# openxrlab/xrsfm

Hardware: AMD Instinct MI355X
Metric: BA iterations/sec x (cams+points) (higher is better)
Workload: dtype f64; 1 GPU; synthetic BAL-style L: 1000 cams / 500000 points / 2000000 obs, GBA accurate (ba_solver.cc:626-629), seed 4; parallelism=single GPU, linear_solver=cholesky (explicit reduced camera matrix, exact)

## Files before the change

### include/xrsfm_ba.h

```cpp
#ifndef XRSFM_BA_H
#define XRSFM_BA_H

#include <stddef.h>
#include <stdint.h>

#ifdef __cplusplus
extern "C" {
#endif

#define XRSFM_BA_VERSION 1

#define XRSFM_BA_OK 0
#define XRSFM_BA_EINVAL (-1)
#define XRSFM_BA_ENODEV (-2)
#define XRSFM_BA_ENOMEM (-3)
#define XRSFM_BA_ECOMM (-4)
#define XRSFM_BA_ESTATE (-5)
#define XRSFM_BA_ETOOBIG (-6)
#define XRSFM_BA_EINTERNAL (-7)
#define XRSFM_BA_ESINGULAR (-8)

#define XRSFM_BA_SIMPLE_PINHOLE 0
#define XRSFM_BA_PINHOLE 1
#define XRSFM_BA_SIMPLE_RADIAL 2
// ... 201 lines not shown
int xrsfm_ba_profile_entry(xrsfm_ba_context *ctx, int index, const char **name, double *total_ms, int *launches);


int xrsfm_ba_debug_linearize(xrsfm_ba_context *ctx, double huber_a, int use_scaling, double *r, double *Jc,
                             double *Jp, double *Hpp, double *gp, double *Hcc_diag, double *gc, double *cost);

int xrsfm_ba_debug_schur_product(xrsfm_ba_context *ctx, double radius, const double *x, double *y, double *b);

int xrsfm_ba_debug_pack(const xrsfm_ba_problem *problem, int32_t stats[8], int32_t *slot_obs);

int xrsfm_ba_debug_sgroup(const xrsfm_ba_problem *problem, int G, int32_t stats[3], int32_t *pos_tile, int32_t *pos_code,
                          int32_t *tile_stride, int32_t *tile_cams, int32_t *tile_cidx, int32_t *cam_ptr_s);
int xrsfm_ba_debug_pack_gram(const xrsfm_ba_problem *problem, int32_t stats[8], int32_t *tile_ncam, uint8_t *slot_cidx,
                             int32_t *slot_campos_g);

int xrsfm_ba_debug_gram_schedule(int n_cams, int32_t *n_inst, int32_t *n_inst_all, uint16_t *entries);

int xrsfm_ba_debug_chol_plan(const xrsfm_ba_problem *problem, int32_t stats[8], int32_t *cam_offset, int32_t *facts);

int xrsfm_ba_debug_device_pack_check(const xrsfm_ba_problem *problem, int32_t *field, int32_t *index);

int xrsfm_ba_debug_set_block_pattern(xrsfm_ba_context *ctx, int n_pairs, const int32_t *row_col);

int xrsfm_ba_debug_cholesky_solve(xrsfm_ba_context *ctx, double radius, double *y, double *S_dense);

int xrsfm_ba_debug_reduced_system(xrsfm_ba_context *ctx, double radius, int32_t facts[16], int32_t *n_blocks, int32_t *blk_rc,
                                  double *blk, double *diag, double *b, double *y);

int xrsfm_ba_debug_wide(xrsfm_ba_context *ctx, double huber_a, double radius, double *cost, double *r, double *Jc, double *Jp,
                        double *Hcc_diag, double *gc, double *y);
// ... 14 lines not shown
```

### xrsfm_amd/capi.py

```python
from __future__ import annotations

import ctypes as C
import os

import numpy as np

from . import _build

_c_double_p = C.POINTER(C.c_double)
_c_int32_p = C.POINTER(C.c_int32)
_c_uint8_p = C.POINTER(C.c_uint8)


class CProblem(C.Structure):
    _fields_ = [
        ("n_cams", C.c_int32), ("n_points", C.c_int32), ("n_obs", C.c_int32), ("n_intr", C.c_int32),
        ("cam_q", _c_double_p), ("cam_t", _c_double_p), ("cam_const", _c_uint8_p), ("cam_intr", _c_int32_p),
        ("intr_model", _c_int32_p), ("intr_params", _c_double_p),
        ("points", _c_double_p), ("point_const", _c_uint8_p),
        ("obs_cam", _c_int32_p), ("obs_pt", _c_int32_p), ("obs_uv", _c_double_p),
    ]


class CPgProblem(C.Structure):
# ... 53 lines not shown
    ]

    def as_dict(self):
        return {f: getattr(self, f) for f, _ in self._fields_}


EXPORTS = [
    "xrsfm_ba_default_options", "xrsfm_ba_version", "xrsfm_ba_create", "xrsfm_ba_comm_unique_id",
    "xrsfm_ba_comm_init", "xrsfm_ba_run", "xrsfm_ba_reset", "xrsfm_ba_download", "xrsfm_ba_destroy",
    "xrsfm_ba_solve", "xrsfm_ba_filter_tracks", "xrsfm_ba_profile_entry", "xrsfm_ba_debug_linearize", "xrsfm_ba_debug_schur_product",
    "xrsfm_ba_debug_cholesky_solve", "xrsfm_ba_debug_set_block_pattern", "xrsfm_ba_debug_pack", "xrsfm_ba_debug_chol_plan", "xrsfm_ba_refine_pose", "xrsfm_ba_refine_pose_options", "xrsfm_ba_debug_comm_hook", "xrsfm_pg_default_options", "xrsfm_pg_solve", "xrsfm_ba_debug_pack_gram", "xrsfm_ba_debug_gram_schedule",
    "xrsfm_tag_default_options", "xrsfm_tag_refine", "xrsfm_ba_refine_poses", "xrsfm_ba_quiesce", "xrsfm_ba_debug_backsub", "xrsfm_ba_device_memory", "xrsfm_ba_download_intrinsics", "xrsfm_ba_debug_wide",
    "xrsfm_ba_debug_device_pack_check", "xrsfm_ba_warmup", "xrsfm_ba_debug_stored_j", "xrsfm_ba_debug_sgroup",
    "xrsfm_ba_debug_reduced_system", "xrsfm_ba_covariance", "xrsfm_ba_point_covariance", "xrsfm_ba_joint_covariance",
    "xrsfm_ba_map_covariance", "xrsfm_ba_debug_backsub_layout", "xrsfm_ba_run_batch", "xrsfm_ba_solve_batch",
    "xrsfm_ba_triangulate_options", "xrsfm_ba_triangulate_tracks",
]

CHOL_FACTS = ("T", "levels", "ordering", "schedule", "macro_levels", "split_levels", "la_depth", "fill_rest", "rest_apart", "packed",
              "bwd", "height_mask", "cw", "blocks", "n", "tiles_nz")
SCHEDULES = ("level", "panel", "lookahead")
BWD_FORMS = ("fused", "per_level", "all", "chunk", "push")


def _facts(v) -> dict:
    f = dict(zip(CHOL_FACTS, (int(x) for x in v)))
    f["schedule"] = SCHEDULES[f["schedule"]]
    f["bwd"] = BWD_FORMS[f["bwd"]]
    f["rest_apart"] = bool(f["rest_apart"]); f["packed"] = bool(f["packed"])
    f["heights"] = sorted(m * f["cw"] for m in range(1, 31) if (f["height_mask"] >> m) & 1)
    return f
# ... 490 lines not shown
          "xrsfm_ba_triangulate_tracks")
    return dict(points=points, status=status, inlier_mask=mask, num_inliers=ninl, num_trials=ntr, best_trial=best)


def debug_pack(problem: ProblemArrays) -> dict:
    stats = np.zeros(8, np.int32)
    slot_obs = np.full(problem.n_obs + 64 * (problem.n_points + 1), -2, np.int32)
    cs = problem.c_struct()
    check(load().xrsfm_ba_debug_pack(C.byref(cs), stats.ctypes.data_as(_c_int32_p), slot_obs.ctypes.data_as(_c_int32_p)), "xrsfm_ba_debug_pack")
    keys = ("tiles", "slots", "items", "regular_tiles", "long_items", "cam_entries", "longest_track", "active_points")
    out = dict(zip(keys, (int(v) for v in stats)))
    out["slot_obs"] = slot_obs[:out["slots"]].copy()
    return out


def debug_device_pack_check(problem: ProblemArrays) -> tuple:
    lib = load()
    lib.xrsfm_ba_debug_device_pack_check.argtypes = [C.POINTER(CProblem), _c_int32_p, _c_int32_p]
    lib.xrsfm_ba_debug_device_pack_check.restype = C.c_int
    f = np.zeros(1, np.int32); i = np.zeros(1, np.int32)
    cs = problem.c_struct()
    check(lib.xrsfm_ba_debug_device_pack_check(C.byref(cs), f.ctypes.data_as(_c_int32_p), i.ctypes.data_as(_c_int32_p)), "xrsfm_ba_debug_device_pack_check")
    return int(f[0]), int(i[0])


def debug_chol_plan(problem: ProblemArrays) -> dict:
    stats = np.zeros(8, np.int32)
    off = np.zeros(max(problem.n_cams, 1), np.int32)
    facts = np.zeros(16, np.int32)
    cs = problem.c_struct()
# ... 171 lines not shown
```

### xrsfm_amd/csrc/ba_chol.h

```cpp
#pragma once
#include "ba_kernels.h"
#include "ba_pack.h"

namespace xba {

constexpr int kNB = 64;
constexpr int kLdT = 66;
constexpr int kCamsPerTileDev = 10;

struct CholDev {
    int n, n_pad, T;
    double* S;
    const int* tmap; size_t ld; size_t tstride;
    double* Linv;
    double* y;
    double* rhs;
    double* x;
    const int* cam_off;
    const int* tile_rows;
    int cw, cpt;
};

__device__ __forceinline__ double* tile_ptr(const CholDev& c, int i, int k) {
    return c.tmap ? c.S + (size_t)c.tmap[i * c.T + k] * c.tstride : c.S + (size_t)(i * kNB) * c.ld + k * kNB;
// ... 286 lines not shown
                   int n_obs_pairs, double* __restrict__ scat2, double radius, double* __restrict__ pair_v = nullptr, int gram4 = 1,
                   const int* __restrict__ sgrp = nullptr, int n_list = 0, int wld = 0) {
    extern __shared__ __attribute__((aligned(16))) double smem_all[];
    constexpr bool MERGED = GRAM && NIK == 0;
    const int lane = MERGED ? (int)__builtin_amdgcn_mbcnt_hi(~0u, __builtin_amdgcn_mbcnt_lo(~0u, 0u)) : (int)threadIdx.x;
    const int wave = MERGED ? __builtin_amdgcn_readfirstlane((int)(threadIdx.x >> 6)) : 0;
    const int pos = MERGED ? (int)blockIdx.x * (int)(blockDim.x >> 6) + wave : (int)blockIdx.x;
    if (MERGED && pos >= n_list) return;
    double* const smem = smem_all + (size_t)wave * wld;
    XBA_STAMP(0, 0);
    SGroup sg{0, 1, smem, wld, 0.0, 0.0, -1};
    if (MERGED && sgrp) {
        const int code = __builtin_amdgcn_readfirstlane(sgrp[pos]);
        sg.idx = code & 15; sg.len = code >> 4;
    }
    const int entry = item_list[MERGED ? n_list - 1 - pos : pos];
    Item it;
    if (GRAM) { it.first_tile = entry; it.n_tiles = 1; }
    else it = d.items[entry];
    if (GRAM || it.n_tiles == 1) {
        int dt0 = -1, dt1 = -1;
        int g4_se = 0, g4_n = 0;
        if (GRAM) {
            const int C0 = d.tile_ncam[it.first_tile];
            const int* src = pair_dst + n_obs_pairs + d.tile_gt_off[it.first_tile];
            const int a0 = lane / kGramTabLd, b0 = lane - kGramTabLd * a0;
            const int a1 = (lane + kWave) / kGramTabLd, b1 = lane + kWave - kGramTabLd * a1;
            if (b0 > a0 && b0 < C0) dt0 = src[a0 * C0 + b0];
            if (b1 > a1 && b1 < C0 && a1 < kGramTabLd) dt1 = src[a1 * C0 + b1];
            if (NIK <= 2 && gram4) g4_se = gram4_sched_load<6>(C0, lane, g4_n);
        }
        const SlotCtx s = load_slot(d, it.first_tile, lane);
        const int cp = d.slot_campos_s[s.slot];
        const int cidx_raw = GRAM ? (int)d.slot_cidx[s.slot] : 0;
        const int L = d.tile_stride[it.first_tile];
        int g_pos = kWave - 1, g_pk0 = 0, g_pk1 = 0, g_pk2 = 0;
        if (GRAM && L == 0) {
            const int C0 = d.tile_ncam[it.first_tile];
            const int* trun = d.tile_run + (size_t)it.first_tile * kTileRunLd;
            const int c0 = lane / 14, c1 = (lane + 64) / 14, c2 = (lane + 128) / 14;
            g_pos = (int)d.slot_gpos[s.slot];
            if (c0 < C0) g_pk0 = trun[c0];
            if (c1 < C0) g_pk1 = trun[c1];
            if (c2 < C0) g_pk2 = trun[c2];
        }
        double V[18];
        int npair = 0, pbase = 0;
        {
            double o28[28];
            XBA_STAMP(0, 1);
            if (s.valid) {
                double hcv[6], gv[3];
                {
// ... 8 lines not shown
                if (PREP) { double hf[6]; point_factor(hcv, radius, hf);
#pragma unroll
                    for (int k = 0; k < 6; ++k) hcv[k] = hf[k]; }
                XBA_STAMP(0, 2);
                pairs_V<PREP>(F, E, hcv, V);
                XBA_STAMP(0, 3);
                pairs_diag<PREP>(F, V, hcv, gv, o28);
            } else if (PREP) { dead_values(V); dead_values(o28); }
            else {
#pragma unroll
                for (int k = 0; k < 18; ++k) V[k] = XBA_DEAD;
#pragma unroll
                for (int k = 0; k < 28; ++k) o28[k] = XBA_DEAD;
            }
            XBA_STAMP(0, 4);
            const int Cg = GRAM ? d.tile_ncam[it.first_tile] : 0;
            if (L > 0) {
                const int T = __popcll(__ballot(s.valid)) / L;
                double* red = smem;
#pragma unroll
                for (int h = 0; h < 2; ++h) {
#pragma unroll
                    for (int k = 0; k < 14; ++k) red[lane * kRedLd + k] = o28[14 * h + k];
                    __builtin_amdgcn_s_waitcnt(0xc07f);
                    __builtin_amdgcn_wave_barrier();
                    if ((L == 4 && T == 16) || (L == 2 && T == 32) || (L == 3 && T == 21)) {
                        const bool on = lane < 14 * L;
                        const int r = on ? lane / 14 : 0, k = lane - 14 * r;
                        const int cpr = __shfl(cp, r, kWave);
                        if (on) {
                            const double* src = red + r * kRedLd + k;
// ... 59 lines not shown
                            }
                            for (; j < n; ++j) sum += src[j * kRedLd];
                            d.scat[28 * (size_t)cpr + 14 * h + k] = sum;
                        }
                    }
                    __builtin_amdgcn_s_waitcnt(0xc07f);
                    __builtin_amdgcn_wave_barrier();
                }
            } else if (cp >= 0) {
                double2* out = reinterpret_cast<double2*>(d.scat + 28 * (size_t)cp);
#pragma unroll
                for (int k = 0; k < 14; ++k) out[k] = make_double2(o28[2 * k], o28[2 * k + 1]);
            }
        }
        XBA_STAMP(0, 5);
        const int C = d.tile_ncam[it.first_tile];
        if (GRAM) {
            const unsigned long long headmask = __ballot(s.head);
            const int T = __popcll(headmask);
            const int nvalid = __popcll(__ballot(s.valid));
            const int t = __popcll(headmask & ((2ull << lane) - 1ull)) - 1;
            const int cidx = s.valid ? cidx_raw : 0;
            int passes = 1;
            (void)gram_lds_need(C, T, &passes);
            const int Th = (T + passes - 1) / passes;
            const int R = 6 * C, Rp = (R + 15) & ~15, Cp = ((3 * Th + 3) & ~3) + kGramPad;
            double* Vst = smem;
            int* dtab = reinterpret_cast<int*>(smem + R * Cp);
            dtab[lane] = dt0;
            if (lane + kWave < kGramTabLd * kGramTabLd) dtab[lane + kWave] = dt1;
            const bool dense = nvalid == T * C;
            (void)Rp;
            unsigned short* sched = reinterpret_cast<unsigned short*>(dtab + kGramTabLd * kGramTabLd);
            if (NIK <= 2 && g4_n > 0 && passes == 1) {
                gram4_sched_store(sched, g4_se, lane, g4_n);
                gram_tile4<6>(Vst, R, Cp, C, dtab, scat2, lane, V, s.valid, t, cidx, T, dense, sched, g4_n, sg, d.scat);
// ... 1294 lines not shown
```

### xrsfm_amd/csrc/ba_kernels.h

```cpp
#pragma once
#include "ba_math.h"

namespace xba {

constexpr int kWave = 64;
constexpr int kBlock = 256;
constexpr int kWavesPerBlock = kBlock / kWave;

struct Item { int first_tile; int n_tiles; };

struct PcgStatus {
    double rz;
    double rr;
    double bb;
    double pq;
    int it;
    int done;
    unsigned arrived;
};

enum Scal {
    S_COST = 0, S_XNORM2_PTS, S_MODEL, S_STEP2_PTS, S_COST_CAND, S_STEP2_CAMS, S_XNORM2_CAMS,
    S_GRADMAX_PTS, S_GRADMAX_CAMS,
    S_BWD_ERR,
// ... 11 lines not shown
struct Dev {
    int n_cams, n_pts, n_tiles, n_slots, n_items;
    const int* slot_cam; const int* slot_pt; const int* slot_campos;
    const double* slot_u; const double* slot_v;
    const Item* items;
    const int* tile_stride;
    const int* tile_maxlen;
    const int* tile_ncam;
    const int* tile_gt_off;
    const unsigned char* slot_cidx;
    const int* slot_campos_g;
    const unsigned char* slot_gpos;
    const int* tile_run;
    const int* cam_ptr_g;
    const int* slot_campos_s; const int* cam_ptr_s;
    CamRec* cam; CamRec* cam_cand; const int* cam_model; const unsigned char* cam_const; const int* cam_ptr;
    double* cam_act;
    double* P; double* P_cand; const unsigned char* pt_const;
    double* scale_c; double* scale_p;
    double* rt; double* Jp;
    double huber_a;
    CamLin* camrec;
    double* Hpp; double* gp; double* Hinv;
    double* Hc;
    double* camlin;
    double* Dc2;
    double* camS;
    double* Minv;
    double* b;
    double* px; double* pr; double* pz; double* pp; double* pq;
    double* yp;
    double* scat;
    double* part;
    double* campart;
    double* ptpart;
    double* pcgpart;
    double* pcgW;
    double* pcgSW;
    double* pcgE;
    double* scal;
    PcgStatus* st;
};

#ifdef XBA_TIMELINE
__device__ unsigned long long g_stamps[3][64][16];
#define XBA_STAMP(kern, i) do { if ((threadIdx.x & 63) == 0 && (blockIdx.x % 97) == 0 && blockIdx.x / 97 < 64 && (threadIdx.x >> 6) == 0) g_stamps[kern][blockIdx.x / 97][i] = __builtin_readcyclecounter(); } while (0)
#define XBA_STAMP_W1(kern, i) do { if ((threadIdx.x & 63) == 0 && (blockIdx.x % 97) == 0 && blockIdx.x / 97 < 64 && (threadIdx.x >> 6) == 1) g_stamps[kern][blockIdx.x / 97][i] = __builtin_readcyclecounter(); } while (0)
#else
#define XBA_STAMP(kern, i) do {} while (0)
#define XBA_STAMP_W1(kern, i) do {} while (0)
#endif

#ifdef XBA_POISON
#define XBA_DEAD (__builtin_nan(""))
#define XBA_DEAD1 (__builtin_nan(""))
#define XBA_DEAD_VALUE(x) ((x) = __builtin_nan(""))
#else
#define XBA_DEAD 0.0
#define XBA_DEAD1 1.0
#define XBA_DEAD_VALUE(x) asm volatile("" : "=v"(x))
// ... 150 lines not shown
    bool valid, head;
};

__device__ __forceinline__ SlotCtx load_slot(const Dev& d, int tile, int lane) {
    SlotCtx s;
    s.lane = lane;
    s.slot = tile * kWave + lane;
    s.cam = d.slot_cam[s.slot];
    s.pt = d.slot_pt[s.slot];
    s.valid = s.cam >= 0;
    const int prev = __shfl_up(s.pt, 1, kWave);
    s.head = s.valid && (lane == 0 || prev != s.pt);
    return s;
}


__device__ __forceinline__ void robust_obs(const double (&M)[9], const double t[3], const double* intr, int model, const double Pw[3],
                                           double u, double v, double huber_a, Proj& pr, double& rho, double& sw) {
    project<true>(M, t, intr, model, Pw, u, v, pr);
    double rho1;
    rho = huber(pr.r0 * pr.r0 + pr.r1 * pr.r1, huber_a, rho1);
    sw = sqrt(rho1);
}

__device__ __forceinline__ void obs_rj(const Dev& d, int slot, int cam, const double (&M)[9], const double Pw[3],
                                       double& r0, double& r1, double (&j)[6]) {
    const CamRec& c = d.cam[cam];
    const double t[3] = {c.t[0], c.t[1], c.t[2]};
    Proj pr;
    double rho, sw;
// ... 83 lines not shown
    extern __shared__ __attribute__((aligned(16))) double lin_smem_acc[];
    double* acc = lin_smem_acc + (threadIdx.x >> 6) * (kWave * 13);
    if (is_long && lane == 0) {
#pragma unroll
        for (int k = 0; k < 9; ++k) acc[k] = 0.0;
    }
    double cost = 0.0, xn2 = 0.0, gm = 0.0;
    int long_pt = -1;
    for (int tl = 0; tl < (LONG ? it.n_tiles : 1); ++tl) {
        const SlotCtx s = load_slot(d, it.first_tile + tl, lane);
        const int cp = d.slot_campos_g[s.slot];
        const int tile = it.first_tile + tl;
        const int stride = d.tile_stride[tile];
        const int Cg = LONG ? 0 : d.tile_ncam[tile];
        const int maxlen = d.tile_maxlen[tile];
        double v[9] = {0, 0, 0, 0, 0, 0, 0, 0, 0};
        double cs[12] = {0, 0, 0, 0, 0, 0, 0, 0, 0, 0, 0, 0};
        double spk[3] = {XBA_DEAD1, XBA_DEAD1, XBA_DEAD1};
        if (s.valid) {
            const CamRec& c = d.cam[s.cam];
            double q[4] = {c.q[0], c.q[1], c.q[2], c.q[3]};
            double t[3] = {c.t[0], c.t[1], c.t[2]};
            const double* P = d.P + 3 * (size_t)s.pt;
            const double Pw[3] = {P[0], P[1], P[2]};
            double M[9];
            quat_to_mat(q, M);
            Proj pr;
            double rho, sw;
            robust_obs(M, t, c.intr, d.cam_model[s.cam], Pw, d.slot_u[s.slot], d.slot_v[s.slot], huber_a, pr, rho, sw);
            cost = cost + rho;
// ... 97 lines not shown
#pragma unroll
            for (int k = 0; k < 9; ++k) acc[k] += v[k];
        }
    }
    if (is_long && lane == 0 && long_pt >= 0) {
        double* H = d.Hpp + 6 * (size_t)long_pt;
#pragma unroll
        for (int k = 0; k < 6; ++k) H[k] = acc[k];
        double* g = d.gp + 3 * (size_t)long_pt;
        g[0] = acc[6]; g[1] = acc[7]; g[2] = acc[8];
        const double* sp = d.scale_p + 3 * (size_t)long_pt;
        gm = fmax(fabs(acc[6] / sp[0]), fmax(fabs(acc[7] / sp[1]), fabs(acc[8] / sp[2])));
    }
    cost = wave_sum(cost);
    xn2 = wave_sum(xn2);
#pragma unroll
    for (int off = 32; off > 0; off >>= 1) gm = fmax(gm, __shfl_xor(gm, off, kWave));
    if (lane == 0) { d.part[item] = cost; d.part[d.n_items + item] = xn2; d.part[2 * (size_t)d.n_items + item] = gm; }
}

__global__ __launch_bounds__(kBlock) __attribute__((amdgpu_waves_per_eu(4, 4))) void k_linearize(Dev d, double huber_a) {
    const int lane = threadIdx.x & (kWave - 1);
    const int item = __builtin_amdgcn_readfirstlane(blockIdx.x * kWavesPerBlock + (threadIdx.x >> 6));
    if (item >= d.n_items) return;
    const Item it = d.items[item];
    if (it.n_tiles > 1) linearize_item<true>(d, it, item, lane, huber_a);
    else linearize_item<false>(d, it, item, lane, huber_a);
}

__global__ __launch_bounds__(kBlock) void k_cost(Dev d, double huber_a) {
    const int lane = threadIdx.x & (kWave - 1);
    const int item = __builtin_amdgcn_readfirstlane(blockIdx.x * kWavesPerBlock + (threadIdx.x >> 6));
    if (item >= d.n_items) return;
    const Item it = d.items[item];
    double cost = 0.0;
    for (int tl = 0; tl < it.n_tiles; ++tl) {
        const int slot = (it.first_tile + tl) * kWave + lane;
        const int cam = d.slot_cam[slot];
        if (cam >= 0) {
            const CamRec& c = d.cam_cand[cam];
            double q[4] = {c.q[0], c.q[1], c.q[2], c.q[3]};
            double t[3] = {c.t[0], c.t[1], c.t[2]};
            const double* P = d.P_cand + 3 * (size_t)d.slot_pt[slot];
            const double Pw[3] = {P[0], P[1], P[2]};
            double M[9];
            quat_to_mat(q, M);
            Proj pr;
            project<false>(M, t, c.intr, d.cam_model[cam], Pw, d.slot_u[slot], d.slot_v[slot], pr);
            double rho1;
            cost += huber(pr.r0 * pr.r0 + pr.r1 * pr.r1, huber_a, rho1);
        }
    }
    cost = wave_sum(cost);
    if (lane == 0) d.part[item] = cost;
}

template <int K, bool WT = false>
__device__ __forceinline__ void segsum_body(const double* __restrict__ scat, const int* __restrict__ ptr, double* __restrict__ out, int c,
// ... 728 lines not shown
template <bool PREP>
#if XBA_BACKSUB_WAVES > 0
__global__ __launch_bounds__(kBlock) __attribute__((amdgpu_waves_per_eu(XBA_BACKSUB_WAVES, XBA_BACKSUB_WAVES)))
#else
__global__ __launch_bounds__(kBlock)
#endif
void k_backsub(Dev d, int n_item_blocks, CamLin* __restrict__ camrec_cand, double radius) {
    if ((int)blockIdx.x >= n_item_blocks) {
        const int c = (blockIdx.x - n_item_blocks) * kBlock + threadIdx.x;
        if (c < d.n_cams) cam_update_one(d, c, d.px + 6 * (size_t)c, camrec_cand);
        return;
    }
    const int lane = threadIdx.x & (kWave - 1);
    const int item = __builtin_amdgcn_readfirstlane(blockIdx.x * kWavesPerBlock + (threadIdx.x >> 6));
    if (item >= d.n_items) return;
    const Item it = d.items[item];
    double model = 0.0, step2 = 0.0;
    if (it.n_tiles == 1) {
        const SlotCtx s = load_slot(d, it.first_tile, lane);
        const int maxlen = d.tile_maxlen[it.first_tile];
        double E[6], v0, v1, r0, r1;
        double w[3] = {0, 0, 0};
        double hh[6], gg[3], spv[3], Pv[3];
        bool var = false;
        if (s.valid) {
            const double* h = (PREP ? d.Hpp : d.Hinv) + 6 * (size_t)s.pt;
            const double* g = d.gp + 3 * (size_t)s.pt;
            const double* sp = d.scale_p + 3 * (size_t)s.pt;
            const double* P = d.P + 3 * (size_t)s.pt;
#pragma unroll
            for (int k = 0; k < 6; ++k) hh[k] = h[k];
            gg[0] = g[0]; gg[1] = g[1]; gg[2] = g[2];
#pragma unroll
            for (int k = 0; k < 3; ++k) { spv[k] = sp[k]; Pv[k] = P[k]; }
            var = !d.pt_const[s.pt];
// ... 100 lines not shown
            if (cam >= 0) {
                const double* y = d.px + 6 * (size_t)cam;
                double F[12], E[6], r0, r1;
                load_FE_rc(d, slot, cam, pt0, F, E, r0, r1);
                double v0 = 0.0, v1 = 0.0;
#pragma unroll
                for (int k = 0; k < 6; ++k) { v0 += F[k] * y[k]; v1 += F[6 + k] * y[k]; }
                const double m0 = v0 + E[0] * u[0] + E[1] * u[1] + E[2] * u[2];
                const double m1 = v1 + E[3] * u[0] + E[4] * u[1] + E[5] * u[2];
                model += m0 * (r0 - 0.5 * m0) + m1 * (r1 - 0.5 * m1);
            }
        }
    }
    model = wave_sum(model);
    step2 = wave_sum(step2);
    if (lane == 0) { d.part[2 * d.n_items + item] = model; d.part[3 * d.n_items + item] = step2; }
}

__global__ void k_cam_update(Dev d) {
    const int c = blockIdx.x * blockDim.x + threadIdx.x;
    if (c >= d.n_cams) return;
    cam_update_one(d, c, d.px + 6 * (size_t)c, nullptr);
}

__device__ __forceinline__ double cam_gradmax_one(const Dev& d, int c, const double* g) {
    double m = 0.0;
    const unsigned cc = d.cam_const[c];
    const bool active = d.cam_act[c] > 0.0;
    const double* sc = d.scale_c + 6 * (size_t)c;
    if (active && !(cc & 1u)) {
// ... 188 lines not shown
```

### xrsfm_amd/csrc/xrsfm_ba.hip

```cpp
#include <dlfcn.h>
#include <hip/hip_runtime.h>

#include <algorithm>
#include <chrono>
#include <condition_variable>
#include <deque>
#include <cmath>
#include <cstdio>
#include <cstdlib>
#include <cstring>
#include <map>
#include <mutex>
#include <thread>
#include <type_traits>
#include <vector>

#include "../../include/xrsfm_ba.h"
#include "ba_chol.h"
#include "ba_cov.h"
#include "ba_filter.h"
#include "ba_kernels.h"
#include "ba_lba.h"
#include "ba_pack.h"
#include "ba_plan.h"
// ... 122 lines not shown
    int n_points_caller = 0;
    double* h_scal = nullptr;
    double* h_scal_dev = nullptr;
    unsigned long long seq = 0;
    PcgStatus* h_st = nullptr;
    void* comm = nullptr; int n_ranks = 1, rank = 0;
    xrsfm_ba_allreduce_fn hook = nullptr; void* hook_user = nullptr; std::vector<double> hook_buf;
    bool multi() const { return comm != nullptr || hook != nullptr; }
    bool profiling = false;
    std::vector<hipEvent_t> ev_pool; size_t ev_used = 0;
    struct Rec { int kid; size_t e0; int tag; };
    std::vector<Rec> recs;
    double prof_ms[K_COUNT] = {0}; int prof_n[K_COUNT] = {0};
    bool dev_packed = false; int host_pack_level = 2;
    int* dpk_slot_obs = nullptr; unsigned char* dpk_gt_cell = nullptr;
    bool linearized = false;
    unsigned long long debug_stall_ticks = 0;
    bool poisoned = false;
    bool fused = true;
    bool wide = false;
    DevW w{};
    std::vector<int> cam_intr_host;
    bool pcg_coarse = true; double* pcg_w = nullptr;
    bool prep_fused = true;
    double step_radius = 0.0;
    bool step_prep = false;
    bool step_valid = false;
    bool backsub_done = false;
    bool gradmax_done = false, published = false;
    double* part2 = nullptr; unsigned* ticket = nullptr;
// ... 515 lines not shown
    (void)hipFuncSetAttribute((const void*)k_schur_pairs<true, false, NI>, hipFuncAttributeMaxDynamicSharedMemorySize, pairs_max);
    XBA_PAIRS_ATTR(1) XBA_PAIRS_ATTR(2) XBA_PAIRS_ATTR(3) XBA_PAIRS_ATTR(4)
#undef XBA_PAIRS_ATTR
    {
        const int merged_max = std::max(pairs_max, kSGroupMax * (kGramSmallLds + 16));
        (void)hipFuncSetAttribute((const void*)k_schur_pairs<true, true, 0>, hipFuncAttributeMaxDynamicSharedMemorySize, merged_max);
        (void)hipFuncSetAttribute((const void*)k_schur_pairs<true, false, 0>, hipFuncAttributeMaxDynamicSharedMemorySize, merged_max);
    }
    (void)hipFuncSetAttribute((const void*)k_schur_pairs<false, true, 0>, hipFuncAttributeMaxDynamicSharedMemorySize, pairs_max);
    (void)hipFuncSetAttribute((const void*)k_schur_pairs<false, false, 0>, hipFuncAttributeMaxDynamicSharedMemorySize, pairs_max);
    (void)hipFuncSetAttribute((const void*)k9_pairs_gram<1>, hipFuncAttributeMaxDynamicSharedMemorySize, pairs_max);
    (void)hipFuncSetAttribute((const void*)k9_pairs_gram<2>, hipFuncAttributeMaxDynamicSharedMemorySize, pairs_max);
    (void)hipFuncSetAttribute((const void*)k9_pairs_gram<3>, hipFuncAttributeMaxDynamicSharedMemorySize, pairs_max);
    (void)hipFuncSetAttribute((const void*)k9_pairs_gram<4>, hipFuncAttributeMaxDynamicSharedMemorySize, pairs_max);
    done_for[device] = 1;
}

int sgroup_setup(xrsfm_ba_context* c, int& n_writes) {
    CholHost& h = c->chol;
    Dev& d = c->d;
    const Packed& k = c->pk;
    d.slot_campos_s = d.slot_campos_g; d.cam_ptr_s = d.cam_ptr_g;
    h.sgroup = 1; h.sgrp = nullptr;
    int G = 4;
    const char* ge = std::getenv("XRSFM_BA_SGROUP");
    if (ge) G = std::atoi(ge);
    G = std::min(G, kSGroupMax);
    int n_merged = 0; size_t shm_merged = 0;
    for (int b = 0; b < 6; ++b) { n_merged += h.gram_n[b]; if (h.gram_n[b] > 0) shm_merged = std::max(shm_merged, h.gram_shm[b]); }
    if (G < 2 || c->wide || !h.gram_merge || n_merged < 2 || shm_merged > (size_t)kGramSmallLds) return 0;
// ... 168 lines not shown
    up.add(&h.tf_ptr, P.tf_ptr); up.add(&h.tf_ent, P.tf_ent);
    up.add(&h.fz_tile, P.fz_tile); up.add(&h.fz_dptr, P.fz_dptr); up.add(&h.fz_dj, P.fz_dj);
    up.add(&h.fz_q, P.fz_q); up.add(&h.fill_rest, P.fill_rest); h.n_fill_rest = (int)P.fill_rest.size();
    up.add(&h.md_tgt, P.md_tgt); up.add(&h.md_q, P.md_q); up.add(&h.md_cj, P.md_cj); up.add(&h.fz_late, P.fz_late);
    h.md_off = P.md_off; h.md_max = P.md_max;
    up.add(&h.tile_cam, P.tile_cam);
    if (dev_keys) h.pairs_items = KR.pairs_items; else up.add(&h.pairs_items, P.pairs_items);
    h.sp_max_chunks = P.sp_max_chunks;
    TRYC(dev_alloc(c, &h.sp_work, (size_t)std::max(1, P.sp_max_chunks) * kPartStride * (P.lookahead ? 2 : (P.la_depth > 0 ? P.la_depth + 1 : 1))));
    if (P.lookahead) TRYC(dev_alloc(c, &h.md_work, (size_t)std::max(1, P.md_max) * kPartStride * 2));
    up.add(&d_cam_off, P.cam_off); up.add(&d_tile_rows, P.tile_rows); up.add(&d_tmap, P.tile_map);
    TRYC(up.flush());
    timer.mark("uploads");
    int n_writes = P.n_writes;
    TRYC(sgroup_setup(c, n_writes));
    const size_t blk_vals = c->wide ? kWB : 36, cam_vals = c->wide ? kWS : 28;
    {
        double* both = nullptr;
        TRYC(dev_alloc(c, &both, (size_t)Nc * cam_vals + (size_t)(P.n_blocks > 0 ? P.n_blocks : 1) * blk_vals));
        if (c->wide) c->w.camS = both; else c->d.camS = both;
        h.Sblk = both + (size_t)Nc * cam_vals;
    }
    {
        const char* g4 = std::getenv("XRSFM_BA_GRAM4");
        h.gram4 = !(g4 && g4[0] == '0');
        const char* pe = std::getenv("XRSFM_BA_PAIR_V");
        h.pair_from_v = !c->wide && h.n_pairs_other > 0 && (pe ? pe[0] != '0' : (P.n_pair_writes >= 262144 && 2LL * P.n_pair_writes >= n_writes));
        const size_t n_scat2 = h.pair_from_v ? (size_t)std::max(0, n_writes - P.n_pair_writes) : (size_t)std::max(0, n_writes);
        TRYC(dev_alloc(c, &h.scat2, std::max<size_t>(1, n_scat2) * blk_vals));
        if (h.pair_from_v) {
// ... 1322 lines not shown
    if (c->wide) {
        TRY(dev_alloc(c, &c->w.Fw, ns * 18)); TRY(dev_alloc(c, &c->w.Ew, ns * 6));
        TRY(dev_alloc(c, &c->w.scale_c, nc * kW)); TRY(dev_alloc(c, &c->w.camlin, nc * 18));
        TRY(dev_alloc(c, &c->w.px, nc * kW + kNB));
        TRY(dev_alloc(c, &c->w.scat, (size_t)(k.n_obs > 0 ? k.n_obs : 1) * kWS));
        c->cam_intr_host.assign(p->cam_intr, p->cam_intr + p->n_cams);
    }
    TRY(dev_alloc(c, &c->part2, (size_t)kTailJobs * kTailGrid));
    TRY(dev_alloc(c, &c->ticket, (size_t)32 * 9));
    {
        unsigned char* gpos = nullptr; int* trun = nullptr;
        TRY(dev_alloc(c, &gpos, ns ? ns : 1)); TRY(dev_alloc(c, &trun, (size_t)std::max(1, k.n_tiles) * kTileRunLd));
        if (k.n_tiles > 0) hipLaunchKernelGGL(k_gram_runs, dim3(cdiv(k.n_tiles, 4)), dim3(256), 0, c->stream, d.slot_cam, d.slot_cidx, d.tile_ncam, k.n_tiles, gpos, trun);
        d.slot_gpos = gpos; d.tile_run = trun;
    }
#undef TRY
    {
        const char* fz = std::getenv("XRSFM_BA_FUSED");
        c->fused = !(fz && fz[0] == '0');
        const char* pf = std::getenv("XRSFM_BA_PREP_FUSED");
        c->prep_fused = !(pf && pf[0] == '0');
        const char* pc = std::getenv("XRSFM_BA_PCG_COARSE");
        c->pcg_coarse = !(pc && pc[0] == '0');
    }
    if (hipMemsetAsync(d.scal, 0, sizeof(double) * S_COUNT, c->stream) != hipSuccess || hipMemsetAsync(d.st, 0, sizeof(PcgStatus), c->stream) != hipSuccess ||
        hipMemsetAsync(c->ticket, 0, sizeof(unsigned) * 32 * 9, c->stream) != hipSuccess ||
        hipStreamSynchronize(c->stream) != hipSuccess) { xrsfm_ba_destroy(c); return XRSFM_BA_ENODEV; }
    timer.mark("work buffers");
    *out = c;
    return XRSFM_BA_OK;
// ... 1219 lines not shown
    std::vector<int> spp;
    PairKeys keyed;
    if ((e = chol_local_keys(k, spp, keyed))) return e == kErrDuplicateObs ? XRSFM_BA_EINVAL : e;
    CholPlan P;
    if ((e = chol_plan_build(k, spp, keyed, nullptr, P, kCholMaxN, kCholMaxBytes))) return e;
    int n_gram = 0, cmax = 0;
    for (int t = 0; t < k.n_tiles; ++t) { n_gram += k.tile_ncam[t] > 0; cmax = std::max(cmax, k.tile_ncam[t]); }
    stats[0] = n_gram; stats[1] = k.n_gt_cells; stats[2] = k.n_cam_entries_g; stats[3] = cmax;
    stats[4] = P.n_pairs_small; stats[5] = P.n_pairs_big; stats[6] = P.n_pairs_other; stats[7] = P.n_writes;
    if (tile_ncam) for (int t = 0; t < k.n_tiles; ++t) tile_ncam[t] = k.tile_ncam[t];
    if (slot_cidx) for (int s2 = 0; s2 < k.n_slots; ++s2) slot_cidx[s2] = k.slot_cidx[s2];
    if (slot_campos_g) for (int s2 = 0; s2 < k.n_slots; ++s2) slot_campos_g[s2] = k.slot_campos_g[s2];
    return 0;
}

int xrsfm_ba_debug_chol_plan(const xrsfm_ba_problem* p, int32_t stats[8], int32_t* cam_offset, int32_t* facts) {
    if (!p || !stats) return XRSFM_BA_EINVAL;
    Packed k;
    const bool wide = problem_is_wide(p);
    int e = pack_problem(*p, k, wide);
    if (e) return e;
    std::vector<int> spp;
    PairKeys keyed;
    if ((e = chol_local_keys(k, spp, keyed))) return e == kErrDuplicateObs ? XRSFM_BA_EINVAL : e;
    CholPlan P;
    if ((e = chol_plan_build(k, spp, keyed, nullptr, P, kCholMaxN, kCholMaxBytes, wide ? kW : 6))) return e == kErrPlanCheck ? XRSFM_BA_EINTERNAL : e;
    stats[0] = P.T; stats[1] = P.n_levels; stats[2] = P.ordering; stats[3] = P.n_hubs; stats[4] = P.band; stats[5] = P.n_blocks;
    stats[6] = (P.use_levels ? 1 : 0) | (P.lookahead ? 2 : 0); stats[7] = P.n_tiles_nz;
    if (cam_offset) for (int i = 0; i < k.n_cams; ++i) cam_offset[i] = P.cam_off[i];
    if (facts) chol_plan_facts(P, facts);
// ... 228 lines not shown
            !cmp(14, k.slot_campos, h.slot_campos) || !cmp(15, k.slot_campos_g, h.slot_campos_g) || !cmp(16, k.cam_ptr, h.cam_ptr) ||
            !cmp(17, k.cam_ptr_g, h.cam_ptr_g) || !cmp(18, k.pt_const, h.pt_const)) return 0;
        {
            const size_t np3 = 3 * (size_t)k.n_pts;
            std::vector<double> P(np3);
            if (np3 && hipMemcpy(P.data(), c->d.P, np3 * sizeof(double), hipMemcpyDeviceToHost) != hipSuccess) return XRSFM_BA_ENODEV;
            for (size_t j = 0; j < (size_t)k.n_pts; ++j)
                for (int a = 0; a < 3; ++a) if (P[3 * j + a] != p->points[3 * (size_t)h.pt_orig[j] + a]) return diff(19, (long long)j);
        }
        return 0;
    });
}

#ifdef XBA_TIMELINE
int xrsfm_ba_debug_stamps(unsigned long long* out) {
    return hipMemcpyFromSymbol(out, HIP_SYMBOL(xba::g_stamps), sizeof(unsigned long long) * 3 * 64 * 16) == hipSuccess ? 0 : XRSFM_BA_ENODEV;
}
#endif

}

int xrsfm_ba_run(xrsfm_ba_context* c, const xrsfm_ba_options* optp, xrsfm_ba_summary* sum) { return no_throw([&] { return ba_run_impl(c, optp, sum); }); }
int xrsfm_ba_run_batch(int32_t n_ctx, xrsfm_ba_context* const* ctxs, const xrsfm_ba_options* opt, xrsfm_ba_summary* summaries, int32_t* codes) {
    return no_throw([&] { return lba_run_batch(n_ctx, ctxs, opt, summaries, codes, nullptr, nullptr); });
}
int xrsfm_ba_solve_batch(const xrsfm_ba_options* opt, int32_t n_problems, xrsfm_ba_problem* problems, xrsfm_ba_summary* summaries, int32_t* codes) {
    return no_throw([&] { return lba_solve_batch(opt, n_problems, problems, summaries, codes); });
}
int xrsfm_ba_covariance(xrsfm_ba_context* c, double huber_a, int32_t n_sel, const int32_t* cam_sel, double* cov) { return no_throw([&] { return covariance_impl(c, huber_a, n_sel, cam_sel, cov); }); }
int xrsfm_ba_point_covariance(xrsfm_ba_context* c, double huber_a, int32_t n_sel, const int32_t* pt_sel, double* cov) { return no_throw([&] { return point_covariance_impl(c, huber_a, n_sel, pt_sel, cov); }); }
int xrsfm_ba_map_covariance(xrsfm_ba_context* c, double huber_a, double* cam_cov, double* pt_cov, uint8_t* cam_status, uint8_t* pt_status) {
// ... 8 lines not shown
```

Before: 1.121 billion cam-pts*iter/s.

## Precompute compact per-tile headers to replace per-lane slot index loads

Adds a 64-byte TileHdr per work item, built on device at setup, that encodes regular tiles (fixed track length up to 8) with the first point, camera list, valid count and a reciprocal for the division. The cost-evaluation, back-substitution and merged Gram/pairs kernels then derive each lane's camera, point, rank and head flag arithmetically from one header load instead of gathering slot_cam, slot_pt, slot_cidx, tile_stride and tile_ncam per lane. Irregular tiles fall back to the old path. It adds setup kernels, extra device memory and more branch complexity, and correctness depends on the header validation logic.

```diff
diff --git a/include/xrsfm_ba.h b/include/xrsfm_ba.h
--- a/include/xrsfm_ba.h
+++ b/include/xrsfm_ba.h
@@ -239,6 +239,9 @@
 int xrsfm_ba_debug_pack_gram(const xrsfm_ba_problem *problem, int32_t stats[8], int32_t *tile_ncam, uint8_t *slot_cidx,
                              int32_t *slot_campos_g);
 
+int xrsfm_ba_debug_tile_headers(const xrsfm_ba_problem *problem, int32_t *n_items, int32_t *headers, int32_t *slot_cam,
+                                int32_t *slot_pt, int32_t *tile_stride);
+
 int xrsfm_ba_debug_gram_schedule(int n_cams, int32_t *n_inst, int32_t *n_inst_all, uint16_t *entries);
 
 int xrsfm_ba_debug_chol_plan(const xrsfm_ba_problem *problem, int32_t stats[8], int32_t *cam_offset, int32_t *facts);
diff --git a/xrsfm_amd/capi.py b/xrsfm_amd/capi.py
--- a/xrsfm_amd/capi.py
+++ b/xrsfm_amd/capi.py
@@ -91,7 +91,7 @@
     "xrsfm_ba_debug_device_pack_check", "xrsfm_ba_warmup", "xrsfm_ba_debug_stored_j", "xrsfm_ba_debug_sgroup",
     "xrsfm_ba_debug_reduced_system", "xrsfm_ba_covariance", "xrsfm_ba_point_covariance", "xrsfm_ba_joint_covariance",
     "xrsfm_ba_map_covariance", "xrsfm_ba_debug_backsub_layout", "xrsfm_ba_run_batch", "xrsfm_ba_solve_batch",
-    "xrsfm_ba_triangulate_options", "xrsfm_ba_triangulate_tracks",
+    "xrsfm_ba_triangulate_options", "xrsfm_ba_triangulate_tracks", "xrsfm_ba_debug_tile_headers",
 ]
 
 CHOL_FACTS = ("T", "levels", "ordering", "schedule", "macro_levels", "split_levels", "la_depth", "fill_rest", "rest_apart", "packed",
@@ -612,6 +612,24 @@
     return out
 
 
+TILE_HDR_FIELDS = ("first_tile", "n_tiles", "L", "inv", "n_valid", "pt0", "maxlen_ncam", "gt_off")
+
+
+def debug_tile_headers(problem: ProblemArrays) -> dict:
+    st = debug_pack(problem)
+    lib = load()
+    lib.xrsfm_ba_debug_tile_headers.argtypes = [C.POINTER(CProblem)] + [_c_int32_p] * 5
+    lib.xrsfm_ba_debug_tile_headers.restype = C.c_int
+    n = np.zeros(1, np.int32)
+    hdr = np.zeros((max(st["items"], 1), 16), np.int32)
+    cam = np.zeros(max(st["slots"], 1), np.int32); pt = np.zeros(max(st["slots"], 1), np.int32); stride = np.zeros(max(st["tiles"], 1), np.int32)
+    cs = problem.c_struct()
+    ip = lambda a: a.ctypes.data_as(_c_int32_p)
+    check(lib.xrsfm_ba_debug_tile_headers(C.byref(cs), ip(n), ip(hdr), ip(cam), ip(pt), ip(stride)), "xrsfm_ba_debug_tile_headers")
+    assert int(n[0]) == st["items"]
+    return dict(headers=hdr[:st["items"]], slot_cam=cam[:st["slots"]], slot_pt=pt[:st["slots"]], tile_stride=stride[:st["tiles"]])
+
+
 def debug_device_pack_check(problem: ProblemArrays) -> tuple:
     lib = load()
     lib.xrsfm_ba_debug_device_pack_check.argtypes = [C.POINTER(CProblem), _c_int32_p, _c_int32_p]
diff --git a/xrsfm_amd/csrc/ba_chol.h b/xrsfm_amd/csrc/ba_chol.h
--- a/xrsfm_amd/csrc/ba_chol.h
+++ b/xrsfm_amd/csrc/ba_chol.h
@@ -324,29 +324,38 @@
         const int code = __builtin_amdgcn_readfirstlane(sgrp[pos]);
         sg.idx = code & 15; sg.len = code >> 4;
     }
-    const int entry = item_list[MERGED ? n_list - 1 - pos : pos];
+    TileHdr hdr;
+    if (MERGED) hdr = load_hdr(d.hdr_gram, pos);
+    const bool fast = MERGED && hdr.L > 0;
     Item it;
-    if (GRAM) { it.first_tile = entry; it.n_tiles = 1; }
-    else it = d.items[entry];
+    if (MERGED) { it.first_tile = hdr.first_tile; it.n_tiles = 1; }
+    else if (GRAM) { it.first_tile = item_list[pos]; it.n_tiles = 1; }
+    else it = d.items[item_list[pos]];
+    const int tile_C = MERGED ? hdr.maxlen_ncam >> 8 : (GRAM ? d.tile_ncam[it.first_tile] : 0);
     if (GRAM || it.n_tiles == 1) {
         int dt0 = -1, dt1 = -1;
         int g4_se = 0, g4_n = 0;
         if (GRAM) {
-            const int C0 = d.tile_ncam[it.first_tile];
-            const int* src = pair_dst + n_obs_pairs + d.tile_gt_off[it.first_tile];
+            const int C0 = tile_C;
+            const int* src = pair_dst + n_obs_pairs + (MERGED ? hdr.gt_off : d.tile_gt_off[it.first_tile]);
             const int a0 = lane / kGramTabLd, b0 = lane - kGramTabLd * a0;
             const int a1 = (lane + kWave) / kGramTabLd, b1 = lane + kWave - kGramTabLd * a1;
             if (b0 > a0 && b0 < C0) dt0 = src[a0 * C0 + b0];
             if (b1 > a1 && b1 < C0 && a1 < kGramTabLd) dt1 = src[a1 * C0 + b1];
             if (NIK <= 2 && gram4) g4_se = gram4_sched_load<6>(C0, lane, g4_n);
         }
-        const SlotCtx s = load_slot(d, it.first_tile, lane);
+        SlotCtx s;
+        int cidx_raw = 0, L;
+        if (fast) { s = load_slot_hdr(hdr, lane, cidx_raw); L = hdr.L; }
+        else {
+            s = load_slot(d, it.first_tile, lane);
+            if (GRAM) cidx_raw = (int)d.slot_cidx[s.slot];
+            L = d.tile_stride[it.first_tile];
+        }
         const int cp = d.slot_campos_s[s.slot];
-        const int cidx_raw = GRAM ? (int)d.slot_cidx[s.slot] : 0;
-        const int L = d.tile_stride[it.first_tile];
         int g_pos = kWave - 1, g_pk0 = 0, g_pk1 = 0, g_pk2 = 0;
         if (GRAM && L == 0) {
-            const int C0 = d.tile_ncam[it.first_tile];
+            const int C0 = tile_C;
             const int* trun = d.tile_run + (size_t)it.first_tile * kTileRunLd;
             const int c0 = lane / 14, c1 = (lane + 64) / 14, c2 = (lane + 128) / 14;
             g_pos = (int)d.slot_gpos[s.slot];
@@ -385,7 +394,7 @@
                 for (int k = 0; k < 28; ++k) o28[k] = XBA_DEAD;
             }
             XBA_STAMP(0, 4);
-            const int Cg = GRAM ? d.tile_ncam[it.first_tile] : 0;
+            const int Cg = tile_C;
             if (L > 0) {
                 const int T = __popcll(__ballot(s.valid)) / L;
                 double* red = smem;
@@ -475,12 +484,18 @@
             }
         }
         XBA_STAMP(0, 5);
-        const int C = d.tile_ncam[it.first_tile];
+        const int C = GRAM ? tile_C : 0;
         if (GRAM) {
-            const unsigned long long headmask = __ballot(s.head);
-            const int T = __popcll(headmask);
-            const int nvalid = __popcll(__ballot(s.valid));
-            const int t = __popcll(headmask & ((2ull << lane) - 1ull)) - 1;
+            int T, nvalid, t;
+            if (fast) {
+                nvalid = hdr.n_valid; T = (nvalid * hdr.inv) >> 9;
+                t = (lane * hdr.inv) >> 9;
+            } else {
+                const unsigned long long headmask = __ballot(s.head);
+                T = __popcll(headmask);
+                nvalid = __popcll(__ballot(s.valid));
+                t = __popcll(headmask & ((2ull << lane) - 1ull)) - 1;
+            }
             const int cidx = s.valid ? cidx_raw : 0;
             int passes = 1;
             (void)gram_lds_need(C, T, &passes);
diff --git a/xrsfm_amd/csrc/ba_kernels.h b/xrsfm_amd/csrc/ba_kernels.h
--- a/xrsfm_amd/csrc/ba_kernels.h
+++ b/xrsfm_amd/csrc/ba_kernels.h
@@ -8,6 +8,19 @@
 constexpr int kWavesPerBlock = kBlock / kWave;
 
 struct Item { int first_tile; int n_tiles; };
+
+constexpr int kHdrMaxL = 8;
+struct __attribute__((aligned(64))) TileHdr {
+    int first_tile, n_tiles;
+    int L;
+    int inv;
+    int n_valid;
+    int pt0;
+    int maxlen_ncam;
+    int gt_off;
+    int cam[kHdrMaxL];
+};
+static_assert(sizeof(TileHdr) == 64, "TileHdr must be one 64-byte line");
 
 struct PcgStatus {
     double rz;
@@ -49,6 +62,7 @@
     const int* tile_run;
     const int* cam_ptr_g;
     const int* slot_campos_s; const int* cam_ptr_s;
+    const TileHdr* hdr_item; const TileHdr* hdr_gram;
     CamRec* cam; CamRec* cam_cand; const int* cam_model; const unsigned char* cam_const; const int* cam_ptr;
     double* cam_act;
     double* P; double* P_cand; const unsigned char* pt_const;
@@ -78,7 +92,7 @@
 };
 
 #ifdef XBA_TIMELINE
-__device__ unsigned long long g_stamps[3][64][16];
+__device__ unsigned long long g_stamps[4][64][16];
 #define XBA_STAMP(kern, i) do { if ((threadIdx.x & 63) == 0 && (blockIdx.x % 97) == 0 && blockIdx.x / 97 < 64 && (threadIdx.x >> 6) == 0) g_stamps[kern][blockIdx.x / 97][i] = __builtin_readcyclecounter(); } while (0)
 #define XBA_STAMP_W1(kern, i) do { if ((threadIdx.x & 63) == 0 && (blockIdx.x % 97) == 0 && blockIdx.x / 97 < 64 && (threadIdx.x >> 6) == 1) g_stamps[kern][blockIdx.x / 97][i] = __builtin_readcyclecounter(); } while (0)
 #else
@@ -259,6 +273,75 @@
     return s;
 }
 
+__host__ __device__ __forceinline__ void hdr_lane_slot(const TileHdr& h, int lane, int& cam, int& pt, int& rank) {
+    const int track = (lane * h.inv) >> 9;
+    rank = lane - track * h.L;
+    const int c0 = h.cam[0], c1 = h.cam[1], c2 = h.cam[2], c3 = h.cam[3], c4 = h.cam[4], c5 = h.cam[5], c6 = h.cam[6], c7 = h.cam[7];
+    int c = c0;
+    c = rank == 1 ? c1 : c; c = rank == 2 ? c2 : c; c = rank == 3 ? c3 : c; c = rank == 4 ? c4 : c;
+    c = rank == 5 ? c5 : c; c = rank == 6 ? c6 : c; c = rank == 7 ? c7 : c;
+    static_assert(kHdrMaxL == 8, "hdr_lane_slot selects among 8 cameras");
+    const bool valid = lane < h.n_valid;
+    cam = valid ? c : -1;
+    pt = valid ? h.pt0 + track : -1;
+}
+__host__ __device__ inline TileHdr tile_header(int first_tile, int n_tiles, bool allow, const int* slot_cam, const int* slot_pt,
+                                               const unsigned char* slot_cidx, const int* tile_stride, const int* tile_maxlen,
+                                               const int* tile_ncam, const int* tile_gt_off) {
+    TileHdr h;
+    h.first_tile = first_tile; h.n_tiles = n_tiles; h.L = 0; h.inv = 0; h.n_valid = 0; h.pt0 = -1;
+    h.maxlen_ncam = tile_maxlen[first_tile] | (tile_ncam[first_tile] << 8);
+    h.gt_off = tile_gt_off[first_tile];
+    for (int r = 0; r < kHdrMaxL; ++r) h.cam[r] = -1;
+    const int L = tile_stride[first_tile], C = tile_ncam[first_tile];
+    if (!allow || n_tiles != 1 || L < 1 || L > kHdrMaxL) return h;
+    const int* sc = slot_cam + (size_t)first_tile * kWave;
+    const int* sp = slot_pt + (size_t)first_tile * kWave;
+    const unsigned char* sx = slot_cidx + (size_t)first_tile * kWave;
+    TileHdr f = h;
+    f.L = L; f.inv = (512 + L - 1) / L; f.pt0 = sp[0];
+    while (f.n_valid < kWave && sc[f.n_valid] >= 0) ++f.n_valid;
+    for (int r = 0; r < L; ++r) f.cam[r] = sc[r];
+    if (C != 0 && C != L) return h;
+    for (int lane = 0; lane < kWave; ++lane) {
+        int cam, pt, rank;
+        hdr_lane_slot(f, lane, cam, pt, rank);
+        if (cam != sc[lane] || pt != sp[lane]) return h;
+        const bool head = cam >= 0 && (lane == 0 || sp[lane - 1] != pt);
+        if (head != (cam >= 0 && rank == 0)) return h;
+        if (C > 0 && cam >= 0 && (int)sx[lane] != rank) return h;
+    }
+    return f;
+}
+__global__ __launch_bounds__(256) void k_tile_headers(const Item* __restrict__ items, const int* __restrict__ list, int n, int allow,
+                                                      const int* __restrict__ slot_cam, const int* __restrict__ slot_pt,
+                                                      const unsigned char* __restrict__ slot_cidx, const int* __restrict__ tile_stride,
+                                                      const int* __restrict__ tile_maxlen, const int* __restrict__ tile_ncam,
+                                                      const int* __restrict__ tile_gt_off, TileHdr* __restrict__ out) {
+    const int p = blockIdx.x * 256 + threadIdx.x;
+    if (p >= n) return;
+    const int first = list ? list[n - 1 - p] : items[p].first_tile;
+    const int nt = list ? 1 : items[p].n_tiles;
+    out[p] = tile_header(first, nt, allow != 0, slot_cam, slot_pt, slot_cidx, tile_stride, tile_maxlen, tile_ncam, tile_gt_off);
+}
+
+__device__ __forceinline__ TileHdr load_hdr(const TileHdr* __restrict__ tab, int i) {
+    const int* __restrict__ w = reinterpret_cast<const int*>(tab + i);
+    TileHdr h;
+    h.first_tile = w[0]; h.n_tiles = w[1]; h.L = w[2]; h.inv = w[3]; h.n_valid = w[4]; h.pt0 = w[5]; h.maxlen_ncam = w[6]; h.gt_off = w[7];
+    h.cam[0] = w[8]; h.cam[1] = w[9]; h.cam[2] = w[10]; h.cam[3] = w[11]; h.cam[4] = w[12]; h.cam[5] = w[13]; h.cam[6] = w[14]; h.cam[7] = w[15];
+    return h;
+}
+__device__ __forceinline__ SlotCtx load_slot_hdr(const TileHdr& h, int lane, int& cidx) {
+    SlotCtx s;
+    s.lane = lane;
+    s.slot = h.first_tile * kWave + lane;
+    hdr_lane_slot(h, lane, s.cam, s.pt, cidx);
+    s.valid = lane < h.n_valid;
+    s.head = s.valid && cidx == 0;
+    return s;
+}
+
 
 __device__ __forceinline__ void robust_obs(const double (&M)[9], const double t[3], const double* intr, int model, const double Pw[3],
                                            double u, double v, double huber_a, Proj& pr, double& rho, double& sw) {
@@ -372,6 +455,7 @@
         const int stride = d.tile_stride[tile];
         const int Cg = LONG ? 0 : d.tile_ncam[tile];
         const int maxlen = d.tile_maxlen[tile];
+        XBA_STAMP(3, 1);
         double v[9] = {0, 0, 0, 0, 0, 0, 0, 0, 0};
         double cs[12] = {0, 0, 0, 0, 0, 0, 0, 0, 0, 0, 0, 0};
         double spk[3] = {XBA_DEAD1, XBA_DEAD1, XBA_DEAD1};
@@ -499,6 +583,7 @@
     }
     cost = wave_sum(cost);
     xn2 = wave_sum(xn2);
+    XBA_STAMP(3, 2);
 #pragma unroll
     for (int off = 32; off > 0; off >>= 1) gm = fmax(gm, __shfl_xor(gm, off, kWave));
     if (lane == 0) { d.part[item] = cost; d.part[d.n_items + item] = xn2; d.part[2 * (size_t)d.n_items + item] = gm; }
@@ -508,6 +593,7 @@
     const int lane = threadIdx.x & (kWave - 1);
     const int item = __builtin_amdgcn_readfirstlane(blockIdx.x * kWavesPerBlock + (threadIdx.x >> 6));
     if (item >= d.n_items) return;
+    XBA_STAMP(3, 0);
     const Item it = d.items[item];
     if (it.n_tiles > 1) linearize_item<true>(d, it, item, lane, huber_a);
     else linearize_item<false>(d, it, item, lane, huber_a);
@@ -517,16 +603,18 @@
     const int lane = threadIdx.x & (kWave - 1);
     const int item = __builtin_amdgcn_readfirstlane(blockIdx.x * kWavesPerBlock + (threadIdx.x >> 6));
     if (item >= d.n_items) return;
-    const Item it = d.items[item];
+    const TileHdr hdr = load_hdr(d.hdr_item, item);
     double cost = 0.0;
-    for (int tl = 0; tl < it.n_tiles; ++tl) {
-        const int slot = (it.first_tile + tl) * kWave + lane;
-        const int cam = d.slot_cam[slot];
+    for (int tl = 0; tl < hdr.n_tiles; ++tl) {
+        const int slot = (hdr.first_tile + tl) * kWave + lane;
+        int cam, pt;
+        if (hdr.L > 0) { int rank; hdr_lane_slot(hdr, lane, cam, pt, rank); }
+        else { cam = d.slot_cam[slot]; pt = d.slot_pt[slot]; }
         if (cam >= 0) {
             const CamRec& c = d.cam_cand[cam];
             double q[4] = {c.q[0], c.q[1], c.q[2], c.q[3]};
             double t[3] = {c.t[0], c.t[1], c.t[2]};
-            const double* P = d.P_cand + 3 * (size_t)d.slot_pt[slot];
+            const double* P = d.P_cand + 3 * (size_t)pt;
             const double Pw[3] = {P[0], P[1], P[2]};
             double M[9];
             quat_to_mat(q, M);
@@ -1285,11 +1373,16 @@
     const int lane = threadIdx.x & (kWave - 1);
     const int item = __builtin_amdgcn_readfirstlane(blockIdx.x * kWavesPerBlock + (threadIdx.x >> 6));
     if (item >= d.n_items) return;
-    const Item it = d.items[item];
+    XBA_STAMP(2, 0);
+    const TileHdr hdr = load_hdr(d.hdr_item, item);
+    const Item it{hdr.first_tile, hdr.n_tiles};
     double model = 0.0, step2 = 0.0;
     if (it.n_tiles == 1) {
-        const SlotCtx s = load_slot(d, it.first_tile, lane);
-        const int maxlen = d.tile_maxlen[it.first_tile];
+        SlotCtx s;
+        int maxlen;
+        if (hdr.L > 0) { int rank; s = load_slot_hdr(hdr, lane, rank); maxlen = hdr.maxlen_ncam & 255; }
+        else { s = load_slot(d, it.first_tile, lane); maxlen = d.tile_maxlen[it.first_tile]; }
+        XBA_STAMP(2, 1);
         double E[6], v0, v1, r0, r1;
         double w[3] = {0, 0, 0};
         double hh[6], gg[3], spv[3], Pv[3];
@@ -1420,6 +1513,7 @@
     }
     model = wave_sum(model);
     step2 = wave_sum(step2);
+    XBA_STAMP(2, 2);
     if (lane == 0) { d.part[2 * d.n_items + item] = model; d.part[3 * d.n_items + item] = step2; }
 }
 
diff --git a/xrsfm_amd/csrc/xrsfm_ba.hip b/xrsfm_amd/csrc/xrsfm_ba.hip
--- a/xrsfm_amd/csrc/xrsfm_ba.hip
+++ b/xrsfm_amd/csrc/xrsfm_ba.hip
@@ -160,6 +160,7 @@
     double prof_ms[K_COUNT] = {0}; int prof_n[K_COUNT] = {0};
     bool dev_packed = false; int host_pack_level = 2;
     int* dpk_slot_obs = nullptr; unsigned char* dpk_gt_cell = nullptr;
+    bool tile_hdr = true;
     bool linearized = false;
     unsigned long long debug_stall_ticks = 0;
     bool poisoned = false;
@@ -705,6 +706,11 @@
     (void)hipFuncSetAttribute((const void*)k9_pairs_gram<3>, hipFuncAttributeMaxDynamicSharedMemorySize, pairs_max);
     (void)hipFuncSetAttribute((const void*)k9_pairs_gram<4>, hipFuncAttributeMaxDynamicSharedMemorySize, pairs_max);
     done_for[device] = 1;
+}
+
+static bool tile_headers_enabled() {
+    const char* e = std::getenv("XRSFM_BA_TILE_HDR");
+    return !(e && e[0] == '0');
 }
 
 int sgroup_setup(xrsfm_ba_context* c, int& n_writes) {
@@ -903,6 +909,20 @@
     timer.mark("uploads");
     int n_writes = P.n_writes;
     TRYC(sgroup_setup(c, n_writes));
+    {
+        int n_merged = 0;
+        for (int b = 0; b < 6; ++b) n_merged += h.gram_n[b];
+        c->d.hdr_gram = nullptr;
+        if (n_merged > 0) {
+            const Dev& d = c->d;
+            TileHdr* hdr = nullptr;
+            TRYC(dev_alloc(c, &hdr, (size_t)n_merged));
+            hipLaunchKernelGGL(k_tile_headers, dim3(cdiv(n_merged, 256)), dim3(256), 0, c->stream, d.items, (const int*)h.pairs_items, n_merged, c->tile_hdr ? 1 : 0,
+                               d.slot_cam, d.slot_pt, d.slot_cidx, d.tile_stride, d.tile_maxlen, d.tile_ncam, d.tile_gt_off, hdr);
+            HIPCHK(hipGetLastError());
+            c->d.hdr_gram = hdr;
+        }
+    }
     const size_t blk_vals = c->wide ? kWB : 36, cam_vals = c->wide ? kWS : 28;
     {
         double* both = nullptr;
@@ -2255,6 +2275,14 @@
         if (k.n_tiles > 0) hipLaunchKernelGGL(k_gram_runs, dim3(cdiv(k.n_tiles, 4)), dim3(256), 0, c->stream, d.slot_cam, d.slot_cidx, d.tile_ncam, k.n_tiles, gpos, trun);
         d.slot_gpos = gpos; d.tile_run = trun;
     }
+    {
+        c->tile_hdr = tile_headers_enabled() && !c->wide;
+        TileHdr* hdr = nullptr;
+        TRY(dev_alloc(c, &hdr, (size_t)std::max(1, d.n_items)));
+        if (d.n_items > 0) hipLaunchKernelGGL(k_tile_headers, dim3(cdiv(d.n_items, 256)), dim3(256), 0, c->stream, d.items, (const int*)nullptr, d.n_items, c->tile_hdr ? 1 : 0,
+                                              d.slot_cam, d.slot_pt, d.slot_cidx, d.tile_stride, d.tile_maxlen, d.tile_ncam, d.tile_gt_off, hdr);
+        d.hdr_item = hdr; d.hdr_gram = nullptr;
+    }
 #undef TRY
     {
         const char* fz = std::getenv("XRSFM_BA_FUSED");
@@ -3504,6 +3532,29 @@
     return 0;
 }
 
+int xrsfm_ba_debug_tile_headers(const xrsfm_ba_problem* p, int32_t* n_items, int32_t* headers, int32_t* slot_cam, int32_t* slot_pt,
+                                int32_t* tile_stride) {
+    if (!p || !n_items) return XRSFM_BA_EINVAL;
+    const bool wide = problem_is_wide(p);
+    Packed k;
+    int e = pack_problem(*p, k, wide);
+    if (e) return e;
+    const int n = (int)k.items.size() / 2;
+    *n_items = n;
+    const bool allow = tile_headers_enabled() && !wide;
+    static_assert(sizeof(TileHdr) == 16 * sizeof(int32_t), "a header is 16 words");
+    if (headers)
+        for (int i = 0; i < n; ++i) {
+            const TileHdr h = tile_header(k.items[2 * i], k.items[2 * i + 1], allow, k.slot_cam.data(), k.slot_pt.data(), k.slot_cidx.data(),
+                                          k.tile_stride.data(), k.tile_maxlen.data(), k.tile_ncam.data(), k.tile_gt_off.data());
+            memcpy(headers + 16 * (size_t)i, &h, sizeof(h));
+        }
+    if (slot_cam) for (int s2 = 0; s2 < k.n_slots; ++s2) slot_cam[s2] = k.slot_cam[s2];
+    if (slot_pt) for (int s2 = 0; s2 < k.n_slots; ++s2) slot_pt[s2] = k.slot_pt[s2];
+    if (tile_stride) for (int t = 0; t < k.n_tiles; ++t) tile_stride[t] = k.tile_stride[t];
+    return 0;
+}
+
 int xrsfm_ba_debug_chol_plan(const xrsfm_ba_problem* p, int32_t stats[8], int32_t* cam_offset, int32_t* facts) {
     if (!p || !stats) return XRSFM_BA_EINVAL;
     Packed k;
@@ -3762,7 +3813,7 @@
 
 #ifdef XBA_TIMELINE
 int xrsfm_ba_debug_stamps(unsigned long long* out) {
-    return hipMemcpyFromSymbol(out, HIP_SYMBOL(xba::g_stamps), sizeof(unsigned long long) * 3 * 64 * 16) == hipSuccess ? 0 : XRSFM_BA_ENODEV;
+    return hipMemcpyFromSymbol(out, HIP_SYMBOL(xba::g_stamps), sizeof(unsigned long long) * 4 * 64 * 16) == hipSuccess ? 0 : XRSFM_BA_ENODEV;
 }
 #endif
 
```

Result: no change. 1.127 billion cam-pts*iter/s (median of 6 runs) (+0.5%).
